# swyoon/Diffusion-by-MaxEntIRL

Hardware: AMD Instinct MI355X
Metric: images/sec (CIFAR-10 DDPM T=10 generation) (higher is better)
Workload: dtype bf16; 1 GPU; CIFAR-10 DDPM U-Net (35.7M params) VARSampler T=10 generation, 256 images/GPU/step, 3x32x32 (BASELINE configs[1]); noise drawn inside the step; global_batch=256, T=10, parallelism=dp1 (independent trajectories, no collective)

## Files before the change

### diffusion-by-maxentirl_amd/csrc/conv1x1_rw.hip

```cpp
#include "conv_common.h"
#include "gn_common.h"

namespace {

#define RW_GPTR(p) ((const __attribute__((address_space(1))) void*)(p))
#define RW_LPTR(p) ((__attribute__((address_space(3))) void*)(p))
#define RW_WAIT_VM(n) asm volatile("s_waitcnt vmcnt(%0)" ::"n"(n) : "memory")
__device__ __forceinline__ void rw_barrier() { asm volatile("s_waitcnt lgkmcnt(0)\n\ts_barrier" ::: "memory"); }

constexpr int RW_CHUNK = 64 * 256;
constexpr int RW_RO = 64 * 256;
constexpr int RW_TBL = 128 * 8;

struct RwGn {
    const float* ab;
    bf16* y;
    int HW, silu;
};

__device__ __forceinline__ void rw_wait_vm(int n) {
    switch (__builtin_amdgcn_readfirstlane(n)) {
#define RW_C(k) case k: RW_WAIT_VM(k); break;
#define RW_C8(k) RW_C(k) RW_C(k + 1) RW_C(k + 2) RW_C(k + 3) RW_C(k + 4) RW_C(k + 5) RW_C(k + 6) RW_C(k + 7)
    RW_C8(0) RW_C8(8) RW_C8(16) RW_C8(24) RW_C8(32) RW_C8(40) RW_C8(48) RW_C8(56)
#undef RW_C8
#undef RW_C
    default: RW_WAIT_VM(0);
    }
}

template <int NCH, int R, bool RES, bool GN>
__global__ __launch_bounds__(256, ((NCH > 3 || R > 4) ? 1 : 2)) void conv1x1_rw_kernel(ConvArgs p, RwGn q) {
    static_assert(R - 1 <= 4 * NCH && R >= 3 && 4 * (R - 2) + 4 * (RES ? 8 : 4) < 64, "ring depth");
    static_assert(!(GN && RES) && (!GN || 5 * (R - 2) + 4 * 4 + 4 * (R - 1) < 64), "GN side output: no residual, vmcnt range");
    constexpr int BOPS = RES ? 8 : 4;
    constexpr int NYOUNG = 4 * (R - 2);
    extern __shared__ __attribute__((aligned(1024))) char smem[];
    char* const ring = smem;

    const int tid = threadIdx.x, lane = tid & 63, h = lane >> 5;
    const int wave = __builtin_amdgcn_readfirstlane(tid >> 6);
    char* const ro = smem + R * RW_CHUNK + wave * 4096;
    char* const tbl = smem + R * RW_CHUNK + RW_RO;
    const int xcd = blockIdx.x & 7, j = blockIdx.x >> 3;
    const int cot = j % p.CT;
    const int nstreams = (gridDim.x >> 3) / p.CT * 8;
    const int stream = (j / p.CT) * 8 + xcd;
    const int ntiles = stream < p.PT ? (p.PT - stream + nstreams - 1) / nstreams : 0;
    if (ntiles == 0) return;

    bf16x8 A[NCH * 8];
    {
        const bf16x8* wf = reinterpret_cast<const bf16x8*>(p.w) + (size_t)(cot * 4 + wave) * 64 + lane;
#pragma unroll
        for (int ks = 0; ks < NCH * 8; ++ks) A[ks] = wf[(size_t)ks * p.CB * 64];
    }
    f32x4 bv[4];
#pragma unroll
    for (int g = 0; g < 4; ++g) {
#pragma unroll
        for (int e = 0; e < 4; ++e) bv[g][e] = 0.f;
        if (p.bias) bv[g] = *reinterpret_cast<const f32x4*>(p.bias + cot * 128 + wave * 32 + 8 * g + 4 * h);
    }
    const float slope = dxmi_act_slope(p.act);

    int dpx[4], ds8[4];
#pragma unroll
    for (int u = 0; u < 4; ++u) {
        dpx[u] = (wave * 4 + u) * 4 + (lane >> 4);
        ds8[u] = ((lane & 15) ^ (dpx[u] & 15)) * 8;
    }
    auto issue_chunk = [&](int tile, int c, int slot) {
        const size_t P0 = (size_t)(stream + tile * nstreams) * 64;
        const int cbase = c * 128;
        const bool first = cbase < p.C0;
        const bf16* src = first ? p.in0 : p.in1;
        const int Cs = first ? p.C0 : p.C1;
        const int coff = first ? cbase : cbase - p.C0;
        if constexpr (GN) {
            const int n = (int)P0 / q.HW;
            __builtin_amdgcn_global_load_lds(RW_GPTR(q.ab + ((size_t)n * (NCH * 128) + cbase) * 2 + wave * 64 + lane),
                                             RW_LPTR(tbl + slot * RW_TBL + wave * 256), 4, 0, 0);
        }
#pragma unroll
        for (int u = 0; u < 4; ++u)
            __builtin_amdgcn_global_load_lds(RW_GPTR(src + (P0 + dpx[u]) * Cs + coff + ds8[u]),
                                             RW_LPTR(ring + slot * RW_CHUNK + (wave * 4 + u) * 1024), 16, 0, 0);
    };
    int rpx[4], rc8[4];
#pragma unroll
    for (int i = 0; i < 4; ++i) {
        rpx[i] = i * 16 + (lane >> 2);
        rc8[i] = ((lane & 3) ^ ((rpx[i] >> 1) & 3)) * 8;
    }
    auto tile_off = [&](int tile, int i) -> size_t {
        return ((size_t)(stream + tile * nstreams) * 64 + rpx[i]) * p.Cout + cot * 128 + wave * 32 + rc8[i];
    };
    auto issue_residual = [&](int tile) {
#pragma unroll
        for (int i = 0; i < 4; ++i)
            __builtin_amdgcn_global_load_lds(RW_GPTR(p.residual + tile_off(tile, i)), RW_LPTR(ro + i * 1024), 16, 0, 0);
    };

    const int gtot = ntiles * NCH;
    if (RES) issue_residual(0);
#pragma unroll
    for (int g = 0; g < R - 1; ++g)
        if (g < gtot) issue_chunk(g / NCH, g % NCH, g);

    int boff[8];
    {
        const int px = lane & 31;
#pragma unroll
        for (int ks = 0; ks < 8; ++ks) boff[ks] = px * 256 + (((ks * 2 + h) ^ (px & 15)) << 4);
    }

    const int gnp = GN ? 4 / p.CT : 0;
    const int gs = tid & 15, gpx0 = cot * (64 / p.CT) + (tid >> 4);

    int slot = 0;
    for (int ti = 0; ti < ntiles; ++ti) {
        f32x16 acc[2];
#pragma unroll
        for (int nb = 0; nb < 2; ++nb)
#pragma unroll
            for (int r = 0; r < 16; ++r) acc[nb][r] = 0.f;
#pragma unroll
        for (int c = 0; c < NCH; ++c) {
            const int g = ti * NCH + c;
            const int kmax = R - 1 - c > 0 ? (R - 1 - c + NCH - 1) / NCH : 0;
            const int nbnd = ti < kmax ? ti : kmax;
            if (g + R - 2 >= gtot) RW_WAIT_VM(0);
            else if (GN) rw_wait_vm(5 * (R - 2) + nbnd * BOPS + (g < R - 1 ? g : R - 1) * gnp);
            else if (nbnd == 0) RW_WAIT_VM(NYOUNG);
            else if (nbnd == 1) RW_WAIT_VM(NYOUNG + BOPS);
            else if (nbnd == 2) RW_WAIT_VM(NYOUNG + 2 * BOPS);
            else if (nbnd == 3) RW_WAIT_VM(NYOUNG + 3 * BOPS);
            else RW_WAIT_VM(NYOUNG + 4 * BOPS);
            rw_barrier();
            {
                const int gi = g + R - 1;
                const int si = slot == 0 ? R - 1 : slot - 1;
                if (gi < gtot) issue_chunk(ti + (c + R - 1) / NCH, (c + R - 1) % NCH, si);
            }
            const char* img = ring + slot * RW_CHUNK;
#pragma unroll
            for (int ks = 0; ks < 8; ++ks)
#pragma unroll
                for (int nb = 0; nb < 2; ++nb) {
                    const bf16x8 b = *reinterpret_cast<const bf16x8*>(img + boff[ks] + nb * (32 * 256));
                    acc[nb] = __builtin_amdgcn_mfma_f32_32x32x16_bf16(A[c * 8 + ks], b, acc[nb], 0, 0, 0);
                }
            if constexpr (GN) {
                float ga[8], gb[8];
                const f32x4* t = reinterpret_cast<const f32x4*>(tbl + slot * RW_TBL + gs * 64);
#pragma unroll
                for (int i = 0; i < 4; ++i) {
                    const f32x4 v = t[i];
                    ga[2 * i] = v[0]; gb[2 * i] = v[1]; ga[2 * i + 1] = v[2]; gb[2 * i + 1] = v[3];
                }
                bf16* const yt = q.y + (size_t)(stream + ti * nstreams) * 64 * (NCH * 128) + c * 128 + gs * 8;
                for (int i = 0; i < gnp; ++i) {
                    const int px = gpx0 + 16 * i;
                    const bf16x8 v = *reinterpret_cast<const bf16x8*>(img + px * 256 + ((gs ^ (px & 15)) << 4));
                    *reinterpret_cast<bf16x8*>(yt + (size_t)px * (NCH * 128)) = gn_norm8(v, ga, gb, q.silu);
                }
            }
            slot = slot + 1 == R ? 0 : slot + 1;
        }
        if (RES) {
            if ((ti + 1) * NCH + R - 1 > gtot) RW_WAIT_VM(0);
            else RW_WAIT_VM(4 * NCH);
        }
#pragma unroll
        for (int nb = 0; nb < 2; ++nb) {
            const int px = nb * 32 + (lane & 31);
#pragma unroll
            for (int g4 = 0; g4 < 4; ++g4) {
                char* a = ro + px * 64 + ((g4 ^ ((px >> 1) & 3)) << 4) + 8 * h;
                f32x4 v;
#pragma unroll
                for (int e = 0; e < 4; ++e) v[e] = acc[nb][4 * g4 + e] + bv[g4][e];
                if (RES) {
                    const bf16x4 r = *reinterpret_cast<const bf16x4*>(a);
#pragma unroll
                    for (int e = 0; e < 4; ++e) v[e] += (float)r[e];
                }
                bf16x4 o;
#pragma unroll
                for (int e = 0; e < 4; ++e) o[e] = (bf16)dxmi_act_lin(v[e], slope);
                *reinterpret_cast<bf16x4*>(a) = o;
            }
        }
        asm volatile("s_waitcnt lgkmcnt(0)" ::: "memory");
        {
            bf16x8 v[4];
#pragma unroll
            for (int i = 0; i < 4; ++i) v[i] = *reinterpret_cast<const bf16x8*>(ro + i * 1024 + lane * 16);
#pragma unroll
            for (int i = 0; i < 4; ++i) *reinterpret_cast<bf16x8*>(reinterpret_cast<bf16*>(p.out) + tile_off(ti, i)) = v[i];
        }
        if (RES && ti + 1 < ntiles) issue_residual(ti + 1);
    }
}

template <int NCH, int R>
int rw_launch(const ConvPlan& p, hipStream_t st) {
    static bool attr_set = false;
    if (!attr_set) {
        (void)hipFuncSetAttribute(reinterpret_cast<const void*>(conv1x1_rw_kernel<NCH, R, true, false>), hipFuncAttributeMaxDynamicSharedMemorySize, 160 * 1024);
        (void)hipFuncSetAttribute(reinterpret_cast<const void*>(conv1x1_rw_kernel<NCH, R, false, false>), hipFuncAttributeMaxDynamicSharedMemorySize, 160 * 1024);
        attr_set = true;
    }
    const RwGn none = {};
    if (p.args.residual) hipLaunchKernelGGL((conv1x1_rw_kernel<NCH, R, true, false>), dim3(p.grid), dim3(256), p.lds, st, p.args, none);
    else hipLaunchKernelGGL((conv1x1_rw_kernel<NCH, R, false, false>), dim3(p.grid), dim3(256), p.lds, st, p.args, none);
    DXMI_CHECK_LAUNCH("dxmi_conv2d_fwd(1x1 rw)");
    return DXMI_OK;
}

template <int NCH, int R>
int rw_launch_gn(const ConvArgs& b, const RwGn& g, int grid, hipStream_t st) {
    const size_t lds = (size_t)R * (RW_CHUNK + RW_TBL) + RW_RO;
    static bool attr_set = false;
    if (!attr_set) {
        (void)hipFuncSetAttribute(reinterpret_cast<const void*>(conv1x1_rw_kernel<NCH, R, false, true>), hipFuncAttributeMaxDynamicSharedMemorySize, 160 * 1024);
        attr_set = true;
    }
    hipLaunchKernelGGL((conv1x1_rw_kernel<NCH, R, false, true>), dim3(grid), dim3(256), lds, st, b, g);
    DXMI_CHECK_LAUNCH("dxmi_groupnorm_silu_shortcut");
    return DXMI_OK;
}

int rw_grid(ConvArgs& b) {
    const int K = b.C0 + b.C1;
    b.PT = (int)((long)b.N * b.OH * b.OW / 64);
    b.CT = b.Cout / 128;
    b.tile_px = 64;
    const int per_xcd = K > 384 ? 32 : 64;
    return 8 * b.CT * (per_xcd / b.CT);
}

}

bool conv1x1_rw_select(const ConvArgs& a, ConvPlan* p) {
    if (a.in_mode != DXMI_IN_NHWC_BF16 || a.out_mode != DXMI_OUT_NHWC_BF16) return false;
    if (a.ksize != 1 || a.stride != 1 || a.pad != 0 || a.ups != 0 || a.mask_src || a.addvec || a.act == DXMI_ACT_SILU) return false;
    const int K = a.C0 + a.C1;
    if (K % 128 != 0 || a.C0 % 128 != 0 || K > 512 || a.Cout % 128 != 0 || a.Cout / 128 > 32) return false;
    const long px = (long)a.N * a.OH * a.OW;
    if (px % 64 != 0 || px / 64 < 512) return false;
    const int nch = K / 128;
    p->kind = ConvKernel::rw; p->t0 = nch; p->t1 = nch > 3 ? 6 : 3;
    p->grid = rw_grid(p->args);
    p->lds = (size_t)p->t1 * RW_CHUNK + RW_RO;
    p->id = 500000 + nch * 1000 + p->t1 * 10 + (a.residual ? 1 : 0);
    return true;
}

int conv1x1_rw_launch(const ConvPlan& p, hipStream_t st) {
    switch (p.t0) {
    case 1: return rw_launch<1, 3>(p, st);
    case 2: return rw_launch<2, 3>(p, st);
    case 3: return rw_launch<3, 3>(p, st);
    default: return rw_launch<4, 6>(p, st);
    }
}

static int gn_shortcut_nch(const dxmi_conv_desc* d, int groups) {
    if (!d || d->ksize != 1 || d->stride != 1 || d->pad != 0 || d->upsample || d->residual || d->addvec || d->mask_src || d->gn_stats ||
        d->gn_out || d->act != DXMI_ACT_NONE || d->variant != 0 || d->in_mode != DXMI_IN_NHWC_BF16 || d->out_mode != DXMI_OUT_NHWC_BF16)
        return 0;
    const int K = d->C0 + d->C1, CT = d->Cout / 128;
    if (d->IH != d->OH || d->IW != d->OW || (d->OH * d->OW) % 64 != 0) return 0;
    if (CT != 1 && CT != 2 && CT != 4) return 0;
    if (groups <= 0 || groups > 32 || K % groups != 0 || (K / groups) % 2 != 0 || d->C1 % 8 != 0) return 0;
    ConvPlan p;
    return conv_plan(d, &p) == DXMI_OK && p.kind == ConvKernel::rw ? p.t0 : 0;
}

extern "C" int dxmi_groupnorm_silu_shortcut_supported(const dxmi_conv_desc* d, int32_t groups) {
    return gn_shortcut_nch(d, groups) > 0 ? 1 : 0;
}

extern "C" int dxmi_groupnorm_silu_shortcut(const dxmi_conv_desc* d, const float* stats0, int32_t P0, const float* stats1, int32_t P1,
                                            const float* gamma, const float* beta, int32_t groups, float eps, int32_t apply_silu, void* y,
                                            float* ab_workspace, void* stream) {
    DXMI_CHECK_ARG(d && d->in0 && d->wpacked && d->out && y && ab_workspace && stats0 && gamma && beta && P0 > 0,
                   "dxmi_groupnorm_silu_shortcut: null pointer");
    DXMI_CHECK_ARG(d->C1 == 0 || (d->in1 && stats1 && P1 > 0), "dxmi_groupnorm_silu_shortcut: C1>0 needs in1 and stats1");
    const int nch = gn_shortcut_nch(d, groups);
    if (nch == 0) return 1;
    const int HW = d->OH * d->OW;
    int rc = gn_finalize_launch(stats0, P0, d->C0, stats1, P1, d->C1, gamma, beta, ab_workspace, d->N, HW, groups, eps, (hipStream_t)stream);
    if (rc != DXMI_OK) return rc;
    ConvArgs b = {};
    b.in0 = (const bf16*)d->in0; b.in1 = (const bf16*)d->in1; b.w = (const bf16*)d->wpacked; b.bias = d->bias; b.out = d->out;
    b.N = d->N; b.IH = d->IH; b.IW = d->IW; b.C0 = d->C0; b.C1 = d->C1; b.OH = d->OH; b.OW = d->OW; b.Cout = d->Cout;
    b.ksize = 1; b.stride = 1; b.act = DXMI_ACT_NONE; b.in_mode = DXMI_IN_NHWC_BF16; b.out_mode = DXMI_OUT_NHWC_BF16;
    b.CB = (d->Cout + 31) / 32;
    const int grid = rw_grid(b);
    const RwGn g = {ab_workspace, (bf16*)y, HW, apply_silu ? 1 : 0};
    const hipStream_t st = (hipStream_t)stream;
    switch (nch) {
    case 1: return rw_launch_gn<1, 3>(b, g, grid, st);
    case 2: return rw_launch_gn<2, 3>(b, g, grid, st);
    case 3: return rw_launch_gn<3, 3>(b, g, grid, st);
    default: return rw_launch_gn<4, 6>(b, g, grid, st);
    }
}
```

Before: 6877 images/s.

## Add 8-wave fused GroupNorm+1x1 shortcut conv kernel for Cout=256

Adds a 512-thread workgroup variant of the fused GroupNorm/SiLU plus 1x1 shortcut convolution kernel. All 256 output channels are covered by one block, with each wave holding its weight slice in registers, a 6-deep LDS ring of input chunks, and a fixed grid of 256 persistent blocks. This is meant to cut redundant input reads across output-channel blocks and improve latency hiding. It is enabled by default through an environment flag for Cout=256 when the channel chunk count is not 2. The cost is a single block per CU with heavy register and LDS use, plus complex vmcnt bookkeeping.

```diff
diff --git a/diffusion-by-maxentirl_amd/csrc/conv1x1_rw.hip b/diffusion-by-maxentirl_amd/csrc/conv1x1_rw.hip
--- a/diffusion-by-maxentirl_amd/csrc/conv1x1_rw.hip
+++ b/diffusion-by-maxentirl_amd/csrc/conv1x1_rw.hip
@@ -202,6 +202,152 @@
         }
         if (RES && ti + 1 < ntiles) issue_residual(ti + 1);
     }
+}
+
+constexpr int RG8_R = 6;
+constexpr int RG8_LDS = RG8_R * (RW_CHUNK + RW_TBL) + 8 * 4096 + 1024;
+
+template <int NCH>
+__global__ __launch_bounds__(512, 1) void conv1x1_rw_gn8_kernel(ConvArgs p, RwGn q) {
+    constexpr int R = RG8_R, GNP = 2, K = NCH * 128;
+    static_assert(3 * (R - 2) + 4 * (R - 1) + GNP * (R - 1) < 64 && RG8_LDS <= 160 * 1024, "vmcnt range, LDS");
+    extern __shared__ __attribute__((aligned(1024))) char smem[];
+    char* const ring = smem;
+
+    const int tid = threadIdx.x, lane = tid & 63, h = lane >> 5;
+    const int wave = __builtin_amdgcn_readfirstlane(tid >> 6);
+    char* const ro = smem + R * RW_CHUNK + wave * 4096;
+    char* const tbl = smem + R * RW_CHUNK + 8 * 4096;
+    float* const btab = reinterpret_cast<float*>(tbl + R * RW_TBL);
+    const int stream = blockIdx.x, nstreams = gridDim.x;
+    const int ntiles = stream < p.PT ? (p.PT - stream + nstreams - 1) / nstreams : 0;
+    if (ntiles == 0) return;
+    const int nd = wave == 0 ? 3 : 2;
+
+    if (tid < 256) btab[tid] = p.bias ? p.bias[tid] : 0.f;
+    bf16x8 A[NCH * 8];
+    {
+        const bf16x8* wf = reinterpret_cast<const bf16x8*>(p.w) + (size_t)wave * 64 + lane;
+#pragma unroll
+        for (int ks = 0; ks < NCH * 8; ++ks) A[ks] = wf[(size_t)ks * p.CB * 64];
+    }
+
+    const int dpx0 = wave * 8 + (lane >> 4);
+    auto issue_chunk = [&](int tile, int c, int slot) {
+        const size_t P0 = (size_t)(stream + tile * nstreams) * 64;
+        const int cbase = c * 128;
+        const bool first = cbase < p.C0;
+        const bf16* src = first ? p.in0 : p.in1;
+        const int Cs = first ? p.C0 : p.C1;
+        const int coff = first ? cbase : cbase - p.C0;
+        if (wave == 0) {
+            const int n = (int)P0 / q.HW;
+            __builtin_amdgcn_global_load_lds(RW_GPTR(q.ab + ((size_t)n * K + cbase) * 2 + lane * 4), RW_LPTR(tbl + slot * RW_TBL), 16, 0, 0);
+        }
+#pragma unroll
+        for (int u = 0; u < 2; ++u) {
+            const int dpx = dpx0 + 4 * u;
+            __builtin_amdgcn_global_load_lds(RW_GPTR(src + (P0 + dpx) * Cs + coff + (((lane & 15) ^ (dpx & 15)) << 3)),
+                                             RW_LPTR(ring + slot * RW_CHUNK + (wave * 2 + u) * 1024), 16, 0, 0);
+        }
+    };
+    const int rpx0 = lane >> 2, rc8 = ((lane & 3) ^ ((lane >> 3) & 3)) * 8;
+
+    const int gtot = ntiles * NCH;
+#pragma unroll
+    for (int g = 0; g < R - 1; ++g)
+        if (g < gtot) issue_chunk(g / NCH, g % NCH, g);
+
+    const int bpx = lane & 31, bsw = bpx & 15;
+    const int brow = bpx * 256;
+    const int gs = tid & 15, gpx = tid >> 4;
+    const int goff = gpx * 256 + ((gs ^ (gpx & 15)) << 4);
+
+    int slot = 0;
+    for (int ti = 0; ti < ntiles; ++ti) {
+        f32x16 acc[2];
+#pragma unroll
+        for (int nb = 0; nb < 2; ++nb)
+#pragma unroll
+            for (int r = 0; r < 16; ++r) acc[nb][r] = 0.f;
+        const size_t P0 = (size_t)(stream + ti * nstreams) * 64;
+#pragma unroll
+        for (int c = 0; c < NCH; ++c) {
+            const int g = ti * NCH + c;
+            const int kmax = R - 1 - c > 0 ? (R - 1 - c + NCH - 1) / NCH : 0;
+            const int nbnd = ti < kmax ? ti : kmax;
+            if (g + R - 2 >= gtot) RW_WAIT_VM(0);
+            else rw_wait_vm(nd * (R - 2) + nbnd * 4 + (g < R - 1 ? g : R - 1) * GNP);
+            rw_barrier();
+            {
+                const int gi = g + R - 1;
+                const int si = slot == 0 ? R - 1 : slot - 1;
+                if (gi < gtot) issue_chunk(ti + (c + R - 1) / NCH, (c + R - 1) % NCH, si);
+            }
+            const char* img = ring + slot * RW_CHUNK;
+#pragma unroll
+            for (int ks = 0; ks < 8; ++ks) {
+                if (ks == 4) __builtin_amdgcn_sched_barrier(0);
+                const int so = ((ks * 2 + h) ^ bsw) << 4;
+#pragma unroll
+                for (int nb = 0; nb < 2; ++nb) {
+                    const bf16x8 b = *reinterpret_cast<const bf16x8*>(img + brow + so + nb * (32 * 256));
+                    acc[nb] = __builtin_amdgcn_mfma_f32_32x32x16_bf16(A[c * 8 + ks], b, acc[nb], 0, 0, 0);
+                }
+            }
+            {
+                float ga[8], gb[8];
+                const f32x4* t = reinterpret_cast<const f32x4*>(tbl + slot * RW_TBL + gs * 64);
+#pragma unroll
+                for (int i = 0; i < 4; ++i) {
+                    const f32x4 v = t[i];
+                    ga[2 * i] = v[0]; gb[2 * i] = v[1]; ga[2 * i + 1] = v[2]; gb[2 * i + 1] = v[3];
+                }
+                bf16* const yt = q.y + (P0 + gpx) * K + c * 128 + gs * 8;
+                bf16x8 v[GNP];
+#pragma unroll
+                for (int i = 0; i < GNP; ++i) v[i] = *reinterpret_cast<const bf16x8*>(img + goff + i * (32 * 256));
+#pragma unroll
+                for (int i = 0; i < GNP; ++i) *reinterpret_cast<bf16x8*>(yt + (size_t)i * 32 * K) = gn_norm8(v[i], ga, gb, q.silu);
+            }
+            slot = slot + 1 == R ? 0 : slot + 1;
+        }
+#pragma unroll
+        for (int nb = 0; nb < 2; ++nb) {
+            const int px = nb * 32 + (lane & 31);
+#pragma unroll
+            for (int g4 = 0; g4 < 4; ++g4) {
+                char* a = ro + px * 64 + ((g4 ^ ((px >> 1) & 3)) << 4) + 8 * h;
+                const f32x4 bv = *reinterpret_cast<const f32x4*>(btab + wave * 32 + 8 * g4 + 4 * h);
+                bf16x4 o;
+#pragma unroll
+                for (int e = 0; e < 4; ++e) o[e] = (bf16)(acc[nb][4 * g4 + e] + bv[e]);
+                *reinterpret_cast<bf16x4*>(a) = o;
+            }
+        }
+        asm volatile("s_waitcnt lgkmcnt(0)" ::: "memory");
+        {
+            bf16x8 v[4];
+#pragma unroll
+            for (int i = 0; i < 4; ++i) v[i] = *reinterpret_cast<const bf16x8*>(ro + i * 1024 + lane * 16);
+            bf16* const ot = reinterpret_cast<bf16*>(p.out) + (P0 + rpx0) * 256 + wave * 32 + rc8;
+#pragma unroll
+            for (int i = 0; i < 4; ++i) *reinterpret_cast<bf16x8*>(ot + (size_t)i * 16 * 256) = v[i];
+        }
+    }
+}
+
+template <int NCH>
+int rw_launch_gn8(ConvArgs b, const RwGn& g, hipStream_t st) {
+    static bool attr_set = false;
+    if (!attr_set) {
+        (void)hipFuncSetAttribute(reinterpret_cast<const void*>(conv1x1_rw_gn8_kernel<NCH>), hipFuncAttributeMaxDynamicSharedMemorySize, 160 * 1024);
+        attr_set = true;
+    }
+    b.CT = 1;
+    hipLaunchKernelGGL((conv1x1_rw_gn8_kernel<NCH>), dim3(256), dim3(512), RG8_LDS, st, b, g);
+    DXMI_CHECK_LAUNCH("dxmi_groupnorm_silu_shortcut");
+    return DXMI_OK;
 }
 
 template <int NCH, int R>
@@ -302,6 +448,14 @@
     const int grid = rw_grid(b);
     const RwGn g = {ab_workspace, (bf16*)y, HW, apply_silu ? 1 : 0};
     const hipStream_t st = (hipStream_t)stream;
+    static const int wg8_env = getenv("DXMI_GN_SHORTCUT_WG8") ? atoi(getenv("DXMI_GN_SHORTCUT_WG8")) : 1;
+    if (wg8_env && d->Cout == 256 && nch != 2) {
+        switch (nch) {
+        case 1: return rw_launch_gn8<1>(b, g, st);
+        case 3: return rw_launch_gn8<3>(b, g, st);
+        default: return rw_launch_gn8<4>(b, g, st);
+        }
+    }
     switch (nch) {
     case 1: return rw_launch_gn<1, 3>(b, g, grid, st);
     case 2: return rw_launch_gn<2, 3>(b, g, grid, st);
```

Result: no change. 6928 images/s, median of 6 (+0.7%).
